# ThibHlln/smartpy

Measured on AMD Instinct MI355X. Metric: MC sample-timesteps/sec/GPU; 1e5 LHS x hourly 10-yr forcing, higher is better.
Workload: dtype f64

## Files before the change

### smartpy_amd/build.py

```python
import os
import shutil
import subprocess
import sys
from concurrent.futures import ThreadPoolExecutor

HERE = os.path.dirname(os.path.abspath(__file__))
CSRC = os.path.join(HERE, 'csrc')
LIB = os.path.join(CSRC, 'libsmart_amd.so')
ARCH = 'gfx950'

UNITS = {
    'smart_literal.hip': ['-ffp-contract=off'],
    'smart_fast_intervals.hip': ['-ffp-contract=fast-honor-pragmas', '-fno-honor-nans'],
    'smart_fast_runs.hip': ['-ffp-contract=fast-honor-pragmas', '-fno-honor-nans'],
    'smart_fast_steps.hip': ['-ffp-contract=fast-honor-pragmas', '-fno-honor-nans'],
    'smart_fast_reports.hip': ['-ffp-contract=fast-honor-pragmas', '-fno-honor-nans'],
    'smart_fast_guarded.hip': ['-ffp-contract=fast-honor-pragmas'],
    'smart_quantiles.hip': [],
    'smart_objfn_windows.hip': [],
    'smart_flow_duration.hip': [],
    'smart_signatures.hip': [],
    'smart_sobol.hip': [],
    'smart_bootstrap.hip': [],
    'smart_pareto.hip': [],
    'smart_ensemble_scores.hip': [],
    'smart_dynia.hip': [],
    'smart_pawn.hip': [],
    'smart_demcz.hip': ['-ffp-contract=off'],
    'smart_error_model.hip': ['-ffp-contract=off'],
    'smart_capi.hip': [],
    'smart_analysis_capi.hip': [],
    'smart_hostio.cpp': ['-pthread'],
}
COMMON = ['-O3', '-fPIC', '-std=c++17', '--offload-arch=' + ARCH, '-fno-gpu-rdc', '-Wall']
DEPS = sorted(f for f in os.listdir(CSRC) if f.endswith('.h')) + [os.path.join('..', '..', 'include', 'smart_amd.h')]


def hipcc():
    exe = shutil.which('hipcc') or '/opt/rocm/bin/hipcc'
    if not os.path.exists(exe):
        raise RuntimeError('hipcc not found: the HIP extension cannot be built')
    return exe


def _stale(target, sources):
    if not os.path.exists(target):
        return True
    t = os.path.getmtime(target)
    return any(os.path.getmtime(s) > t for s in sources)


def build(force=False, verbose=False, extra_flags=(), lib_path=LIB):
    cc = hipcc()
    deps = [os.path.join(CSRC, d) for d in DEPS] + [os.path.abspath(__file__)]
    objs, jobs = [], []
    suffix = '' if lib_path == LIB else '.' + os.path.basename(lib_path)
    for unit, flags in UNITS.items():
        src = os.path.join(CSRC, unit)
        obj = os.path.join(CSRC, os.path.splitext(unit)[0] + suffix + '.o')
        if force or _stale(obj, [src] + deps):
            jobs.append([cc] + COMMON + flags + list(extra_flags) + ['-c', src, '-o', obj])
        objs.append(obj)
    if jobs:
        if verbose:
            for cmd in jobs:
                print(' '.join(cmd))
        with ThreadPoolExecutor(max_workers=min(len(jobs), os.cpu_count() or 1)) as pool:
            list(pool.map(subprocess.check_call, jobs))
    from . import isa_lint
    relink = force or _stale(lib_path, objs)
    if relink or isa_lint.record_state(lib_path) != 'this-build':
        tmp = '%s.%d.tmp' % (lib_path, os.getpid())
        try:
            if relink:
                cmd = [cc, '-shared', '-fPIC', '-pthread', '--offload-arch=' + ARCH, '-o', tmp] + objs
                if verbose:
                    print(' '.join(cmd))
                subprocess.check_call(cmd)
            else:
                shutil.copy(lib_path, tmp)
            isa_lint.lint_and_record(tmp, record_for=lib_path, stamp=True, check=lambda path: lint(path, verbose))
            os.replace(tmp, lib_path)
        finally:
            if os.path.exists(tmp):
                os.remove(tmp)
    return lib_path


class BuildLintError(RuntimeError):
    pass


def lint(path, verbose=False):
    from . import isa_lint
    report = isa_lint.check_library(path)
    report['library'] = os.path.basename(LIB)
    if verbose or report['problems']:
# ... 11 lines not shown
```

### smartpy_amd/csrc/smart_capi.hip

```cpp
#include "smart_capi_internal.h"
#include "smart_fast_entry.h"

#include <cmath>
#include <cstdarg>
#include <cstdio>
#include <cstdlib>
#include <cstring>
#include <mutex>
#include <vector>

namespace smart {

static_assert(kStatusSliceTimeout == SMART_STATUS_SLICE_TIMEOUT && kStatusStalePlan == SMART_STATUS_STALE_PLAN,
              "status bits of smart_device.h and include/smart_amd.h");

static thread_local char g_err[512] = "";

int fail(int code, const char *fmt, ...)
{
    va_list ap;
    va_start(ap, fmt);
    vsnprintf(g_err, sizeof(g_err), fmt, ap);
    va_end(ap);
    return code;
// ... 56 lines not shown
                    r[4 * j + 1] = f[t].y;
                    r[4 * j + 2] = obs && dev && rr >= 0 && rr < a.R ? obs[rr] : 0.0;
                    r[4 * j + 3] = obs && dev && rr >= 0 && rr < a.R ? dev[rr] : 0.0;
                }
                code = a.gap == 1 ? every_code(p, step_kind(f[2 * p]), step_kind(f[2 * p + 1]))
                                  : gap_code(p, a.gap, step_kind(f[2 * p]), step_kind(f[2 * p + 1]));
            }
            for (int j = 0; j < 8; ++j)
                rec[p * 8 + j] = r[j];
            codes[p] = code;
        }
    }
    if (bad)
        __hip_atomic_fetch_or(a.fflags + blockIdx.y, bad, __ATOMIC_RELAXED, __HIP_MEMORY_SCOPE_AGENT);
    if (wild && a.hdr)
        __hip_atomic_fetch_or(a.hdr + kHdrStatus, kStatusNonFiniteForcing, __ATOMIC_RELAXED, __HIP_MEMORY_SCOPE_AGENT);
}

__global__ void smart_workspace_reset(int *hdr, long n_hdr, int *flags, long n_flags)
{
    const long i = (long)blockIdx.x * blockDim.x + threadIdx.x;
    if (i < n_hdr)
        hdr[i] = 0;
    if (i < n_flags)
        flags[i] = 0;
}

__global__ __launch_bounds__(kWave) void smart_classify_rows(KArgs a)
{
    const int cls = wave_class(a, (long)blockIdx.x, (long)blockIdx.y);
    if (threadIdx.x == 0) {
        __hip_atomic_fetch_or(a.hdr + kHdrPlan, 1 << cls, __ATOMIC_RELAXED, __HIP_MEMORY_SCOPE_AGENT);
        if (cls == 3)
            __hip_atomic_fetch_add(a.hdr + kHdrPlanIllCond, 1, __ATOMIC_RELAXED, __HIP_MEMORY_SCOPE_AGENT);
    }
}

__global__ void smart_classify_forcing(KArgs a, int *hdr)
{
    const long c = (long)blockIdx.x * blockDim.x + threadIdx.x;
    if (c < a.n_catch) {
        const int kind = forcing_kind(a, a.fflags[c]);
        __hip_atomic_fetch_or(hdr + kHdrPlan,
                              kind == kForcingIntervals ? SMART_PLAN_FORCING_PIECEWISE
                                                        : (kind == kForcingRuns ? SMART_PLAN_FORCING_RUNS
                                                                                : SMART_PLAN_FORCING_VARYING),
                              __ATOMIC_RELAXED, __HIP_MEMORY_SCOPE_AGENT);
    }
}

constexpr int kMaxDevices = 64, kMaxTodo = 8, kMaxAux = kMaxTodo - 1;

struct DeviceCtx {
    std::once_flag once;
    int n_simd = 0;
    std::mutex mu;
    hipStream_t aux[kMaxAux] = {};
    hipEvent_t fork = nullptr, join[kMaxAux] = {};
    size_t lds_size[kNumFastKernels][17] = {};
    bool lds_known[kNumFastKernels][17] = {};
};

static DeviceCtx g_dev[kMaxDevices];

static DeviceCtx *device_ctx()
{
    int dev = 0;
    if (hipGetDevice(&dev) != hipSuccess || dev < 0 || dev >= kMaxDevices)
        return nullptr;
    DeviceCtx *d = &g_dev[dev];
    std::call_once(d->once, [d, dev] {
        int cus = 0;
        if (hipDeviceGetAttribute(&cus, hipDeviceAttributeMultiprocessorCount, dev) == hipSuccess && cus > 0)
            d->n_simd = cus * 4;
    });
    return d->n_simd > 0 ? d : nullptr;
}

struct Overrides {
    int pair_blocks = -1;
    int time_slices = 0;
    int illcond_form = SMART_LITERAL_FORM_AUTO;
    bool taper = true;
    int exits = -1;
    long max_polls = kDefaultMaxPolls;
    int drop_slice = 0;
    bool allsteps_fast = false;
};

static Overrides read_overrides()
{
    Overrides o;
    if (const char *v = getenv("SMART_PAIR_BLOCKS"))
        o.pair_blocks = atoi(v) != 0;
    if (const char *v = getenv("SMART_TIME_SLICES"))
        o.time_slices = atoi(v) <= 0 ? 1 : atoi(v);
    if (const char *v = getenv("SMART_SLICE_TAPER"))
        o.taper = atoi(v) != 0;
    if (const char *v = getenv("SMART_ILLCOND_FORM"))
        o.illcond_form = !strcmp(v, "rows")    ? SMART_LITERAL_FORM_ROWS
                         : !strcmp(v, "lanes") ? SMART_LITERAL_FORM_LANES
                                               : SMART_LITERAL_FORM_AUTO;
    if (const char *v = getenv("SMART_EXITS"))
        o.exits = atoi(v) != 0;
    if (const char *v = getenv("SMART_DEBUG_MAX_POLLS"))
        o.max_polls = atol(v) > 0 ? atol(v) : kDefaultMaxPolls;
    if (const char *v = getenv("SMART_DEBUG_DROP_SLICE"))
        o.drop_slice = atoi(v);
    if (const char *v = getenv("SMART_ALLSTEPS_MATH"))
        o.allsteps_fast = !strcmp(v, "fast");
    return o;
}

struct FastKernelInfo {
    const void *handle;
    const char *name;
    int cls;
    bool sliced;
    int waves;
};

static const FastKernelInfo kFastKernels[kNumFastKernels] = {
#define X(id, symbol, cls, sliced, waves) {reinterpret_cast<const void *>(&symbol), #symbol, cls, sliced, waves},
    SMART_FAST_KERNELS(X)
#undef X
};

static size_t lds_for_residency(DeviceCtx *d, FastKernel k, int per_cu)
{
    if (per_cu < 1 || per_cu > 16)
        return 0;
    if (!d->lds_known[k][per_cu]) {
        size_t found = 0;
        for (size_t x = (size_t)(160 * 1024 / per_cu) / 256 * 256;
             x >= 1024 && x > (size_t)(160 * 1024 / (per_cu + 1)) - 2048; x -= 256) {
            int nb = 0;
            if (hipOccupancyMaxActiveBlocksPerMultiprocessor(&nb, kFastKernels[k].handle, kWave, x) != hipSuccess)
                break;
            if (nb == per_cu) {
                found = x;
                break;
            }
            if (nb > per_cu)
                break;
        }
        d->lds_size[k][per_cu] = found;
        d->lds_known[k][per_cu] = true;
    }
    return d->lds_size[k][per_cu];
}

static int merged_report(const SmartEnsemble *e);

extern "C" __attribute__((used, visibility("default"))) volatile char smart_lint_stamp[40] = "SMART_LINT_STAMP=unchecked";

static bool pair_blocks_wanted(const Overrides &ov)
{
    if (ov.pair_blocks >= 0)
        return ov.pair_blocks != 0;
    static const char ok[] = "SMART_LINT_STAMP=pairs-ok";
    for (size_t i = 0; i + 1 < sizeof(ok); ++i)
        if (smart_lint_stamp[i] != ok[i])
            return false;
    return true;
}

static bool uses_records(const SmartEnsemble *e)
{
    const int merged = merged_report(e);
    return merged == kReportEvery || ((merged == kReportMean || merged == kReportLast) && e->report_gap % kChunk != 0);
}

struct Layout {
    size_t header = 0;
    size_t stats_off = 0, stats = 0;
    size_t state_off = 0, state = 0;
    size_t flags_off = 0, flags = 0;
    size_t codes_off = 0, codes = 0;
    size_t ecodes_off = 0;
#ifdef SMART_SLICE_TIMELINE
    size_t timeline_off = 0, timeline = 0;
#endif
    size_t total = 0;
    size_t handover() const { return state + flags; }
};
// ... 303 lines not shown
    x.n_seg = plan_time_slices(e, d->n_simd, ov, &x.per_simd, &x.load);
    if (x.n_seg > 1 && !w.state)
        x.n_seg = 1;
    x.exits = ov.exits >= 0 ? ov.exits : x.load > 2.5;
    x.class_mask = plan & 0xf;
    if (plan & SMART_PLAN_CLASS_REGULAR) {
        if (x.intervals) {
            if (plan & SMART_PLAN_FORCING_PIECEWISE) {
                x.push(e->final_vars ? kIntervalsStates : (x.exits ? kIntervalsExits : kIntervals));
                x.pc_mask |= kPcIntervals;
            }
            if (plan & SMART_PLAN_FORCING_RUNS) {
                x.push(e->final_vars ? kRunsStates : (x.exits ? kRunsExits : kRuns));
                x.pc_mask |= kPcRuns;
            }
            if (plan & SMART_PLAN_FORCING_VARYING) {
                x.push(e->final_vars ? kStepsStates : kSteps);
                x.pc_mask |= kPcSteps;
            }
        } else if (x.report == kReportLast) {
            if (plan & SMART_PLAN_FORCING_PIECEWISE) {
                x.push(kIntervalsRaw);
                x.pc_mask |= kPcIntervals;
            }
            if (plan & (SMART_PLAN_FORCING_RUNS | SMART_PLAN_FORCING_VARYING)) {
                x.push(kStepsRaw);
                x.pc_mask |= kPcSteps | kPcRuns;
            }
        } else if (x.report == kReportEvery) {
            x.push(kStepsEvery);
            x.pc_mask = kPcIntervals | kPcSteps | kPcRuns;
        } else {
            x.push(kPlain);
        }
    }
    if (plan & SMART_PLAN_CLASS_STIFF)
        x.push(kStiff);
    if (plan & SMART_PLAN_CLASS_GUARD)
        x.push(kGuard);
    if (plan & SMART_PLAN_CLASS_ILLCOND) {
        x.illcond_blocks = count_illcond_blocks(e, plan);
        x.illcond_rows = illcond_form(e, d->n_simd, x.illcond_blocks, ov);
        x.push(x.illcond_rows ? kIllCond : kIllCondLanes);
    }
    if (x.overflow)
        return fail(SMART_E_SIZE, "internal: a call wants more than %d kernels", kMaxTodo);
    if (x.n_todo == 0)
        return fail(SMART_E_SIZE, "the plan names no class of rows");
    return SMART_OK;
}

static int run(const SmartEnsemble *e, const Overrides &ov, bool literal_rows = false)
{
    int rc = check(e);
    if (rc)
        return rc;
    if ((rc = device_ready()))
        return rc;
    hipStream_t s = (hipStream_t)e->stream;
    const Workspace w = carve(e, ov);
    KArgs a = kernel_args(e, w);

    if (e->objfn)
        hipLaunchKernelGGL(smart_obs_prepare, dim3((unsigned)e->n_catchments), dim3(256), 0, s, e->obs, a.R, w.stats);

    const dim3 grid((unsigned)a.n_blocks, (unsigned)e->n_catchments);
    if (e->math_mode == SMART_MATH_LITERAL) {
        if (w.hdr)
            reset_workspace(w, e->n_catchments, nullptr, 0, s);
        a.hdr = nullptr;
        launch_literal(a, grid, a.np_mean ? (size_t)a.gap * kWave * sizeof(double) : 0, s, literal_rows);
        HIP_TRY(hipGetLastError());
        return SMART_OK;
    }

    DeviceCtx *d = device_ctx();
    if (!d)
        return fail(SMART_E_NO_DEVICE, "cannot query the current HIP device");
    Decision x;
    if ((rc = decide(e, d, w, ov, &x)))
        return rc;
    const int n_seg = x.n_seg, n_todo = x.n_todo;
    a.exits = x.exits;
    a.class_mask = x.class_mask;
    a.pc_mask = x.pc_mask;

    KArgs a_sliced = a;
    if (n_seg > 1) {
        a_sliced.n_seg = n_seg;
        a_sliced.taper = ov.taper && slice_taper_applies(a.W / a.gap + a.R, n_seg);
        a_sliced.seg_state = (double *)w.state;
        a_sliced.seg_flag = (int *)(w.state + (w.lay.flags_off - w.lay.state_off));
        a_sliced.max_polls = ov.max_polls;
        a_sliced.debug_drop = ov.drop_slice;
#ifdef SMART_SLICE_TIMELINE
        a_sliced.timeline = (unsigned long long *)w.timeline;
#endif
    }
    if (w.hdr) {
        reset_workspace(w, e->n_catchments, a_sliced.seg_flag, n_seg > 1 ? a.seg_blocks : 0, s);
        scan_forcing(e, a, w, ov, s);
        if (x.report >= 0 && (x.class_mask & SMART_PLAN_CLASS_REGULAR)) {
            a.fflags = a_sliced.fflags = w.fflags;
            set_codes(&a, w, ov);
            a_sliced.codes = a.codes, a_sliced.estream = a.estream, a_sliced.ecodes = a.ecodes;
        }
    }

    std::lock_guard<std::mutex> lock(d->mu);
    auto launch = [&](FastKernel k, hipStream_t st) -> hipError_t {
        if (kFastKernels[k].sliced && n_seg > 1) {
            const size_t lds = x.per_simd <= 3 ? lds_for_residency(d, k, 4 * x.per_simd) : 0;
            return launch_kernel(k, a_sliced, dim3((unsigned)(a.seg_blocks * n_seg), 1), lds, st);
        }
        return launch_kernel(k, a, dim3(grid.x * kFastKernels[k].waves, grid.y), 0, st);
    };
    if (n_todo == 1) {
        HIP_TRY(launch(x.todo[0], s));
        return SMART_OK;
    }
    if (!d->fork) {
        HIP_TRY(hipEventCreateWithFlags(&d->fork, hipEventDisableTiming));
        for (int i = 0; i < kMaxAux; ++i) {
            HIP_TRY(hipStreamCreateWithFlags(&d->aux[i], hipStreamNonBlocking));
            HIP_TRY(hipEventCreateWithFlags(&d->join[i], hipEventDisableTiming));
        }
    }
    HIP_TRY(hipEventRecord(d->fork, s));
    for (int i = 1; i < n_todo; ++i) {
        HIP_TRY(hipStreamWaitEvent(d->aux[i - 1], d->fork, 0));
        HIP_TRY(launch(x.todo[i], d->aux[i - 1]));
        HIP_TRY(hipEventRecord(d->join[i - 1], d->aux[i - 1]));
    }
    HIP_TRY(launch(x.todo[0], s));
    for (int i = 1; i < n_todo; ++i)
        HIP_TRY(hipStreamWaitEvent(s, d->join[i - 1], 0));
    return SMART_OK;
}

static int describe(const SmartEnsemble *e, const Overrides &ov, char *text, int64_t len)
{
    if (!text || len < 1)
        return fail(SMART_E_NULL, "smart_describe_launch: no room for the text");
    text[0] = 0;
    int rc = check(e);
    if (rc)
        return rc;
    if (e->math_mode == SMART_MATH_LITERAL) {
        snprintf(text, (size_t)len, "smart_ensemble_literal");
        return SMART_OK;
    }
    if ((rc = device_ready()))
        return rc;
    DeviceCtx *d = device_ctx();
    if (!d)
        return fail(SMART_E_NO_DEVICE, "cannot query the current HIP device");
    Decision x;
    if ((rc = decide(e, d, carve(e, ov), ov, &x)))
        return rc;
    const long blocks = (e->n_samples + kWave - 1) / kWave * e->n_catchments;
    size_t used = 0;
    for (int i = 0; i < x.n_todo && used + 1 < (size_t)len; ++i) {
        const FastKernelInfo &k = kFastKernels[x.todo[i]];
        char *at = text + used;
        const size_t room = (size_t)len - used;
        int n;
// ... 419 lines not shown
```

### smartpy_amd/csrc/smart_device.h

```cpp
#pragma once

#include "smart_slice_cuts.h"
#include "smart_matrix_common.h"

#include <hip/hip_runtime.h>

#include <type_traits>

namespace smart {

constexpr int kMaxDiv = 12;
constexpr int kForcingInsane = 1 << 30;

struct KArgs {
    long N, T, W, gap, R, first_len;
    int report_type;
    int np_mean;
    double dt;
    const double *area;
    const double *forcing;
    const double *params;
    long pstride_c;
    const double *extra;
    const double *initial;
    const double *obs;
    const double *gw_obs;
    const double *ws;
    double *discharge;
    long ld;
    double *gw;
    double *objfn;
    double *final_vars;
    int exits = 1;
    int class_mask = 0xf;
    int pc_mask = 0x7;
    int *hdr = nullptr;
    int *fflags = nullptr;
    const double *estream = nullptr;
    const unsigned *ecodes = nullptr;
    int pair_stride = 0;
    const uint2 *codes = nullptr;
    int n_div = 0;
    int div[kMaxDiv] = {};
    int n_seg = 1;
    int taper = 0;
    long n_catch = 1;
    long n_blocks = 0;
    long seg_blocks = 0;
    double *seg_state = nullptr;
    int *seg_flag = nullptr;
    long max_polls = 0;
    int debug_drop = 0;
#ifdef SMART_SLICE_TIMELINE
    unsigned long long *timeline = nullptr;
#endif
};
#ifdef SMART_SLICE_TIMELINE
constexpr int kTimelineFields = 5, kTimelineSlices = 64;
__device__ __forceinline__ void timeline_note(const KArgs &a, long block, long c, int seg, int field,
                                              unsigned long long value)
{
    if (a.timeline && a.n_seg > 1 && seg < kTimelineSlices && seg < a.n_seg && threadIdx.x == 0)
        a.timeline[((long)seg * a.seg_blocks + c * a.n_blocks + block) * kTimelineFields + field] = value;
}
#endif

enum SegField : int {
    kSegState = 0,
    kSegDenRaw = 13,
    kSegPend = 15,
    kSegOutflows = 16,
    kSegA = 17,
    kSegB,
    kSegC1,
    kSegC2,
    kSegC3,
    kSegShift,
    kSegFields
};
enum HdrInt : int {
    kHdrStatus = 0,
    kHdrTicket = 1,
    kHdrPlan = 8,
    kHdrPlanIllCond = 9,
    kHdrInts = 64
};
constexpr int kStatusSliceTimeout = 1, kStatusStalePlan = 2, kStatusNonFiniteForcing = 4;

__device__ __forceinline__ void raise_status(const KArgs &a, int bit)
{
    if (a.hdr && threadIdx.x == 0)
        __hip_atomic_fetch_or(a.hdr + kHdrStatus, bit, __ATOMIC_RELAXED, __HIP_MEMORY_SCOPE_AGENT);
}

#define SMART_NOPS_0 ""
#define SMART_NOPS_1 "s_nop 0\n\t"
#define SMART_NOPS_2 SMART_NOPS_1 SMART_NOPS_1
#define SMART_NOPS_4 SMART_NOPS_2 SMART_NOPS_2
#define SMART_NOPS_8 SMART_NOPS_4 SMART_NOPS_4
#define SMART_NOPS_3 SMART_NOPS_2 SMART_NOPS_1
#define SMART_NOPS_5 SMART_NOPS_4 SMART_NOPS_1
#define SMART_NOPS_6 SMART_NOPS_4 SMART_NOPS_2
#define SMART_NOPS_7 SMART_NOPS_4 SMART_NOPS_3
#define SMART_NOPS_9 SMART_NOPS_8 SMART_NOPS_1
#define SMART_NOPS_10 SMART_NOPS_8 SMART_NOPS_2
#define SMART_NOPS_11 SMART_NOPS_8 SMART_NOPS_3
#define SMART_NOPS_12 SMART_NOPS_8 SMART_NOPS_4
#define SMART_NOPS_13 SMART_NOPS_8 SMART_NOPS_5
#define SMART_NOPS_14 SMART_NOPS_8 SMART_NOPS_6
#define SMART_NOPS_15 SMART_NOPS_8 SMART_NOPS_7
#define SMART_NOPS_(n) SMART_NOPS_##n
#define SMART_NOPS(n) SMART_NOPS_(n)
#define SMART_PLACE_LOOP(phase) asm volatile(".p2align 6\n\t" SMART_NOPS(phase))
#ifndef SMART_STEPS_PHASE
#define SMART_STEPS_PHASE 1
#endif
#ifndef SMART_PS_STRIDE
#define SMART_PS_STRIDE 2368
// ... 844 lines not shown
__device__ __forceinline__ Work claim_work(const KArgs &a, int sliced_kernel)
{
    Work w;
    if (a.n_seg > 1) {
        unsigned t = 0;
        if (threadIdx.x == 0)
            t = __hip_atomic_fetch_add(reinterpret_cast<unsigned *>(a.hdr) + kHdrTicket + sliced_kernel, 1u,
                                       __ATOMIC_RELAXED, __HIP_MEMORY_SCOPE_AGENT);
        t = (unsigned)__builtin_amdgcn_readfirstlane((int)t);
        const long slot = (long)(t % (unsigned long)a.seg_blocks);
        w.seg = (int)(t / (unsigned long)a.seg_blocks);
        w.c = slot / a.n_blocks;
        w.block = slot % a.n_blocks;
    } else {
        w.block = blockIdx.x;
        w.c = blockIdx.y;
        w.seg = 0;
    }
    return w;
}

__device__ __forceinline__ bool wait_for_slice(const KArgs &a, long slot, int seg)
{
    int *flag = a.seg_flag + slot;
    long polls = 0;
    int v;
    while ((v = __hip_atomic_load(flag, __ATOMIC_RELAXED, __HIP_MEMORY_SCOPE_AGENT)) > -seg && v < seg) {
        __builtin_amdgcn_s_sleep(kPollSleep);
        if (++polls > a.max_polls) {
            raise_status(a, kStatusSliceTimeout);
            return false;
        }
    }
    __builtin_amdgcn_fence(__ATOMIC_ACQUIRE, "agent");
    return v >= seg;
}

__device__ __forceinline__ void publish_slice(const KArgs &a, long slot, int seg, bool good)
{
    asm volatile("s_waitcnt vmcnt(0)" ::: "memory");
    __builtin_amdgcn_fence(__ATOMIC_RELEASE, "agent");
    asm volatile("s_waitcnt vmcnt(0)" ::: "memory");
    if (threadIdx.x == 0)
        __hip_atomic_store(a.seg_flag + slot, good ? seg + 1 : -(seg + 1), __ATOMIC_RELAXED, __HIP_MEMORY_SCOPE_AGENT);
}

constexpr int kReportMean = 0, kReportLast = 1, kReportEvery = 2;

template <class Model, int FORCING, int REPORT = kReportMean>
__device__ __forceinline__ void run_ensemble_merged(const KArgs &a, const double2 *__restrict__ forcing,
                                                    const double *__restrict__ obs_all,
                                                    const double *__restrict__ ws_all, long block, long catchment,
                                                    int seg, int fflags)
{
    constexpr bool piecewise = FORCING != kForcingVarying;
    constexpr bool runs = FORCING == kForcingRuns;
    static_assert(REPORT == kReportMean || (!Model::kSplit && !runs), "raw / every-step reports: merged model, no runs");
    static_assert(REPORT != kReportEvery || !piecewise, "a report every step is a step loop");
    static_assert(Model::kStateFields <= kSegPend, "the model's states end in front of the other hand-over fields");
    const LaneCtx x = lane_ctx(a, block, catchment);
    const long slot = catchment * a.n_blocks + block;
    Model m;
    init_model(a, x, m);
    const long gap = a.gap;
    const long run_len = runs ? run_length(a, fflags) : gap;
    if constexpr (piecewise)
        m.setup_intervals(REPORT == kReportLast ? run_len - 1 : run_len);
    const double2 *__restrict__ f = forcing + x.c * a.T;

    int fits = 0;
    unsigned not_quick = ~0u;
    if constexpr (piecewise && Model::kWetAsm) {
        m.note_capacity();
        const bool fits_b = m.over_mask == 0;
        fits = __builtin_amdgcn_readfirstlane((int)fits_b);
        not_quick = 0u - (unsigned)__builtin_amdgcn_readfirstlane((int)!(fits_b && !(fflags & kForcingInsane)));
        asm("" : "+s"(fits), "+s"(not_quick));
    }
    auto no_bits = [](double x, unsigned unless = 0) {
        unsigned long long b = __builtin_bit_cast(unsigned long long, x) | unless;
        asm("" : "+s"(b));
        return b == 0;
    };
    auto interval = [&](const double2 v, double &acc, double &num, double &den) {
        if constexpr (piecewise && Model::kWetAsm) {
            if (no_bits(v.x, not_quick)) {
                if (no_bits(v.y)) {
                    m.calm_interval(run_len, acc);
                } else {
                    m.dry_interval(-v.y, run_len, acc);
                }
                return;
            }
        }
        const double ex = m.excess(v.x, v.y);
        if (ex < 0.0) {
            m.dry_interval(ex, run_len, acc);
        } else {
            if constexpr (piecewise && Model::kWetAsm)
                m.wet_interval(ex, run_len, acc, num, den, fits);
            else
                m.wet_interval(ex, run_len, acc, num, den);
        }
    };

    [[maybe_unused]] auto interval_last = [&](const double2 v, double &qo, double &qg, double &qi) {
        if constexpr (piecewise && REPORT == kReportLast && Model::kWetAsm) {
            double sink = 0.0, n0 = 0.0, n1 = 0.0;
            if (no_bits(v.x, not_quick)) {
                if (no_bits(v.y)) {
                    m.calm_interval(gap - 1, sink);
                    m.last_step_flows(qo, qg, qi);
                    m.calm_interval(1, sink);
                } else {
                    m.dry_interval_last(-v.y, gap, qo, qg, qi);
                }
                return;
            }
            const double ex = m.excess(v.x, v.y);
            if (ex < 0.0) {
                m.dry_interval_last(ex, gap, qo, qg, qi);
            } else {
                m.wet_interval(ex, gap - 1, sink, n0, n1, fits);
                m.last_step_flows(qo, qg, qi);
                m.wet_interval(ex, 1, sink, n0, n1, fits);
            }
        }
    };

    const long n_warm = a.W / gap, n_all = n_warm + a.R;
    const long g0 = a.taper ? slice_cut_tapered(n_all, seg, a.n_seg) : n_all * seg / a.n_seg;
    const long g1 = a.taper ? slice_cut_tapered(n_all, seg + 1, a.n_seg) : n_all * (seg + 1) / a.n_seg;
    const long wa = g0 < n_warm ? g0 : n_warm, wb = g1 < n_warm ? g1 : n_warm;
    const long ra = g0 > n_warm ? g0 - n_warm : 0, rb = g1 > n_warm ? g1 - n_warm : 0;
    const bool last = seg == a.n_seg - 1;

    Reporter rep;
    rep.init(a, x, obs_all, ws_all);
    [[maybe_unused]] const double *__restrict__ obs_c = obs_all ? obs_all + x.c * a.R : nullptr;
    [[maybe_unused]] const double *__restrict__ dev_c = ws_all ? ws_all + x.c * (kWsHead + a.R) + kWsHead : nullptr;
    [[maybe_unused]] const uint2 *codes_c = a.codes ? a.codes + x.c * code_chunks(a.T) : nullptr;
    [[maybe_unused]] const double2 *f_asm = reinterpret_cast<const double2 *>(a.forcing) + x.c * a.T;
    double num = 0.0, den = 0.0, q_out_total = 0.0;
    [[maybe_unused]] double num_raw = 0.0, den_raw = 0.0;
    double *hand = a.seg_state + (slot * kSegFields) * kWave + x.lane;
    if (seg > 0) {
        if (!wait_for_slice(a, slot, seg)) {
            const double nan = quiet_nan();
            if (a.discharge && x.live)
                for (long r = ra; r < rb; ++r)
                    a.discharge[(x.c * a.R + r) * a.ld + x.n] = nan;
            if (last) {
                if (x.live) {
                    a.gw[x.c * a.N + x.n] = nan;
                    if (a.objfn)
                        for (int i = 0; i < 8; ++i)
                            a.objfn[(x.c * a.N + x.n) * 8 + i] = nan;
                    if (a.final_vars)
                        for (int i = 0; i < 19; ++i)
                            a.final_vars[(x.c * a.N + x.n) * 19 + i] = nan;
                }
            } else {
                publish_slice(a, slot, seg, false);
            }
            return;
        }
#ifdef SMART_SLICE_TIMELINE
        timeline_note(a, block, catchment, seg, 3, __builtin_amdgcn_s_memrealtime());
#endif
        m.load_state(hand, kWave);
        if constexpr (REPORT == kReportLast) {
            num_raw = hand[kSegOutflows * kWave];
            den_raw = hand[kSegDenRaw * kWave];
        } else {
            q_out_total = hand[kSegOutflows * kWave];
        }
        rep.A = hand[kSegA * kWave];
        rep.B = hand[kSegB * kWave];
        rep.C1 = hand[kSegC1 * kWave];
        rep.C2 = hand[kSegC2 * kWave];
        rep.C3 = hand[kSegC3 * kWave];
        rep.shift = hand[kSegShift * kWave];
    }

    double *const park = Model::kSplit ? a.final_vars + (x.c * a.N + x.n) * 19 : nullptr;
    auto park_state = [&]() {
        if constexpr (Model::kSplit) {
            m.save_state(park, 1);
            if constexpr (!piecewise)
                park[15] = m.pend;
        }
    };

    double s0 = 0.0, s1 = 0.0, s2 = 0.0;
    const double inv_gap = 1.0 / (double)gap;
    const bool starts_run = ra == 0 && (rb > 0 || last);
    constexpr bool deferring = !piecewise;
    [[maybe_unused]] const int n_lead = (int)(rep.r1 + 1 > ra ? (rep.r1 + 1 < rb ? rep.r1 + 1 - ra : rb - ra) : 0);
    [[maybe_unused]] int store = __builtin_amdgcn_readfirstlane((int)(a.discharge != nullptr));
    asm("" : "+s"(store));
    [[maybe_unused]] const int k_park = Model::kSplit && ra <= a.R - 1 && a.R - 1 < rb ? (int)(a.R - 1 - ra) : -1;
    if constexpr (piecewise)
        rep.begin_rows(a, x, ra);
    if constexpr (runs) {
        const long per = gap / run_len;
        interval_loop(f, wa * per, wb * per, run_len, [&](int, const double2 v) { interval(v, s0, s1, s2); });
        if (starts_run)
            m.begin_run();
// ... 318 lines not shown
```

### smartpy_amd/csrc/smart_fast_model.h

```cpp
#pragma once

#include "smart_device.h"
#include "smart_fast_arms.h"

namespace smart {

template <bool STIFF, bool GUARD, bool MERGE = false, bool EXITS = true, bool SPLIT = false>
struct FastModel {
    static_assert(!(MERGE && STIFF), "the clamps of structure.py:429-450 act on each reservoir separately");
    static_assert(MERGE || !SPLIT, "SPLIT refines the merged form");
    static constexpr bool kExactDivide = false;
    static constexpr bool kSplit = SPLIT;

    double pT, pC, pD, hz, sz, z;
    double dec_s, dec_f, dec_g, cq_s, cq_f, cq_g;
    double a_r, inv_a_r;
    double a_s, a_f, a_g;
    double car_s, car_f, car_g, om_ar;
    double k_s, k_f, k_g, k_r, mm_to_m3;
    double l0, l1, l2, l3, l4, l5;
    double u_ove, u_dra, u_int, u_sgw, u_dgw, u_riv;
    double q_out, q_in, q_gw;

    __device__ void setup(double area, double dt, const double *p)
// ... 288 lines not shown
        l1 = fma(-l1, s1 * 0.5, l1);
        l2 = fma(-l2, s1 * (1.0 / 3.0), l2);
        l3 = fma(-l3, s1 * 0.25, l3);
        l4 = fma(-l4, s1 * 0.2, l4);
        l5 = fma(-l5, s1 * (1.0 / 6.0), l5);
        const double deep = SPLIT ? deep_leak(s1, p2, p3, p4, p5, p6) : 0.0;
        l0 = fma(-l0, p6, l0);
        l1 = fma(-l1, p5, l1);
        l2 = fma(-l2, p4, l2);
        l3 = fma(-l3, p3, l3);
        l4 = fma(-l4, p2, l4);
        l5 = fma(-l5, s1, l5);
        const double inf = (tot - after_int) + fma(-pD, rem, ex_in);
        fma_in_place(u_ove, dec_s, fma(pD, rem, e_h * tot));
        fma_in_place(u_int, dec_f, inf);
        const double upper = (l0 + l1) + (l2 + l3), lower = l4 + l5;
        asm("v_add_f64 %0, %1, %2" : "+v"(tot) : "v"(upper), "v"(lower));
        const double xg = after_int - tot;
        fma_in_place(u_sgw, dec_g, xg);
        if (SPLIT) {
            fma_in_place(u_dra, dec_s, pD * rem);
            fma_in_place(u_dgw, dec_g, deep);
        }
        if (kBalanceSums)
            xg_sum += xg;
    }

#ifndef SMART_WET_ASM
#define SMART_WET_ASM 1
#endif
    static constexpr bool kWetAsm = SMART_WET_ASM && kLeakBalance && !kExits && !SPLIT && !STIFF;

    __device__ __forceinline__ void calm_interval(long n, double &acc)
    {
        static_assert(kWetAsm, "calm_interval() is the asm loop of the straight-line merged kernels");
        double tot = layer_sum();
        double t0, t1, xf, xg, w_s1, w_p2, w_p3, w_p4, w_p5, w_p6, w_ai;
        int cnt;
        asm volatile(SMART_A_CALM_INTERVAL
                     : [l0] "+v"(l0), [l1] "+v"(l1), [l2] "+v"(l2), [l3] "+v"(l3), [l4] "+v"(l4), [l5] "+v"(l5),
                       [ys] "+v"(u_ove), [yf] "+v"(u_int), [yg] "+v"(u_sgw), [riv] "+v"(u_riv), [acc] "+v"(acc),
                       [tot] "+v"(tot), [xgs] "+v"(xg_sum), [t0] "=&v"(t0), [t1] "=&v"(t1), [xf] "=&v"(xf),
                       [xg] "=&v"(xg), [s1] "=&v"(w_s1), [p2] "=&v"(w_p2), [p3] "=&v"(w_p3), [p4] "=&v"(w_p4),
                       [p5] "=&v"(w_p5), [p6] "=&v"(w_p6), [ai] "=&v"(w_ai), [cnt] "=&s"(cnt)
                     : [cs] "v"(car_s), [cf] "v"(car_f), [cg] "v"(car_g), [oma] "v"(om_ar), [ds] "v"(dec_s),
                       [df] "v"(dec_f), [dg] "v"(dec_g), [sz] "v"(sz), [k3] "s"(-(1.0 / 3.0)), [k5] "s"(-0.2),
                       [k6] "s"(-(1.0 / 6.0)), [n] "s"((int)n)
                     : "scc");
    }

    __device__ __forceinline__ void wet_interval(double ex, long n, double &acc, double &num, double &den,
                                                 const int fits = 0)
    {
        if constexpr (kWetAsm) {
            const double e_h = ex * hz;
            double tot = layer_sum();
            double t0, t1, xs, xf, xg, w_s1, w_p2, w_p3, w_p4, w_p5, w_p6, w_ai;
            int cnt;
            asm volatile(SMART_A_WET_INTERVAL
                         : [l0] "+v"(l0), [l1] "+v"(l1), [l2] "+v"(l2), [l3] "+v"(l3), [l4] "+v"(l4), [l5] "+v"(l5),
                           [ys] "+v"(u_ove), [yf] "+v"(u_int), [yg] "+v"(u_sgw), [riv] "+v"(u_riv), [acc] "+v"(acc),
                           [tot] "+v"(tot), [xgs] "+v"(xg_sum), [t0] "=&v"(t0), [t1] "=&v"(t1), [xs] "=&v"(xs),
                           [xf] "=&v"(xf), [xg] "=&v"(xg), [s1] "=&v"(w_s1), [p2] "=&v"(w_p2), [p3] "=&v"(w_p3),
                           [p4] "=&v"(w_p4), [p5] "=&v"(w_p5), [p6] "=&v"(w_p6), [ai] "=&v"(w_ai), [cnt] "=&s"(cnt)
                         : [cs] "v"(car_s), [cf] "v"(car_f), [cg] "v"(car_g), [oma] "v"(om_ar), [ds] "v"(dec_s),
                           [df] "v"(dec_f), [dg] "v"(dec_g), [sz] "v"(sz), [z] "v"(z), [pd] "v"(pD), [ex] "v"(ex),
                           [eh] "v"(e_h), [k3] "s"(-(1.0 / 3.0)), [k5] "s"(-0.2), [k6] "s"(-(1.0 / 6.0)),
                           [n] "s"((int)n), [ok] "s"(fits)
                         : "scc", "vcc");
        } else if (kLeakBalance) {
            const double e_h = ex * hz;
            double tot = layer_sum();
#pragma unroll 1
            for (long k = 0; k < n; ++k) {
                route_and_sum(acc, num, den);
                wet_balance(ex, e_h, tot);
            }
        } else {
            for (long k = 0; k < n; ++k) {
                route_and_sum(acc, num, den);
                wet_lanes(ex);
            }
        }
    }

    __device__ __forceinline__ void dry_lanes(double ex)
    {
        double d = -ex;
        dry(l0, d, pC);
        auto handed_down = [](double x) { return GUARD ? x != 0.0 : x > 0.0; };
        if (__builtin_amdgcn_ballot_w64(handed_down(d)) != 0) {
            dry(l1, d, pC);
            if (__builtin_amdgcn_ballot_w64(handed_down(d)) != 0) {
                dry(l2, d, pC);
                dry(l3, d, pC);
                dry(l4, d, pC);
                dry(l5, d, pC);
            }
        }
        u_ove = clamp(u_ove * dec_s);
        u_int = clamp(u_int * dec_f);
        u_sgw = clamp(u_sgw * dec_g);
        if (!MERGE || SPLIT) {
            u_dra = clamp(u_dra * dec_s);
            u_dgw = clamp(u_dgw * dec_g);
        }
    }

    __device__ __forceinline__ void route_and_sum(double &acc, double &num, double &den)
    {
        double q_r = u_riv;
        double u_new;
        if (MERGE && !STIFF && kBalanceSums) {
            q_out = u_riv;
            q_gw = cq_g * u_sgw;
            q_in = fma(cq_s, u_ove, fma(cq_f, u_int, q_gw));
            const double y = fma(car_s, u_ove, fma(car_f, u_int, car_g * u_sgw));
            if (kExits) {
                sum_then_fma_in_place(acc, u_riv, om_ar, y);
            } else {
                acc += u_riv;
                fma_in_place(u_riv, om_ar, y);
            }
            return;
        }
        if (MERGE) {
            u_new = u_riv;
            fma_in_place(u_new, om_ar, fma(car_s, u_ove, fma(car_f, u_int, car_g * u_sgw)));
            q_gw = cq_g * u_sgw;
            q_in = fma(cq_s, u_ove, fma(cq_f, u_int, q_gw));
        } else {
            q_gw = u_sgw + u_dgw;
            q_in = ((u_ove + u_dra) + u_int) + q_gw;
            u_new = fma(q_in - u_riv, a_r, u_riv);
        }
        if (STIFF) {
            if (u_new < 0.0) {
                q_r = 0.95 * fma(u_riv, inv_a_r, q_in);
                u_new = fma(q_in - q_r, a_r, u_riv);
            }
        }
        u_riv = u_new;
        q_out = q_r;
        acc += q_r;
        if (!kBalanceSums) {
            num += q_gw;
            den += q_in;
        }
    }

    static constexpr int kStateFields = 15;

    __device__ void save_state(double *p, int stride) const
    {
        const double v[kStateFields] = {l0, l1, l2, l3, l4, l5, u_ove, u_int, u_sgw, u_riv, g0, r0, xg_sum, u_dra, u_dgw};
#pragma unroll
        for (int i = 0; i < (SPLIT ? 15 : 13); ++i)
            p[i * stride] = v[i];
    }

    __device__ void load_state(const double *p, int stride)
    {
        double v[kStateFields] = {};
#pragma unroll
        for (int i = 0; i < (SPLIT ? 15 : 13); ++i)
            v[i] = p[i * stride];
// ... 513 lines not shown
```

### smartpy_amd/csrc/smart_fast_reports.hip

```cpp
#include "smart_fast_entry.h"

namespace smart {

SMART_FAST_KERNEL(smart_fast_steps_raw) { merged_kernel<FastModel<false, false, true>, kForcingVarying, kReportLast>(a, forcing, obs, ws); }

SMART_FAST_KERNEL(smart_fast_intervals_raw)
{
    merged_kernel<FastModel<false, false, true, false>, kForcingIntervals, kReportLast>(a, forcing, obs, ws);
}

SMART_FAST_KERNEL(smart_fast_steps_every) { merged_kernel<FastModel<false, false, true>, kForcingVarying, kReportEvery>(a, forcing, obs, ws); }

}
```

### smartpy_amd/csrc/smart_fast_runs.hip

```cpp
#include "smart_fast_entry.h"

namespace smart {

SMART_FAST_KERNEL(smart_fast_runs_exits) { merged_kernel<FastModel<false, false, true, true>, kForcingRuns>(a, forcing, obs, ws); }

SMART_FAST_KERNEL(smart_fast_runs) { merged_kernel<FastModel<false, false, true, false>, kForcingRuns>(a, forcing, obs, ws); }

SMART_FAST_KERNEL(smart_fast_runs_states)
{
    merged_kernel<FastModel<false, false, true, true, true>, kForcingRuns>(a, forcing, obs, ws);
}

}
```

Before: 959.6 billion.

## Make wet/dry interval branching wave-uniform with twin-state merge for mixed waves

Replaces the per-lane wet/dry branch in the runs and interval-last paths with a wave ballot. Uniform waves take a single path, and mixed waves run both paths on a copied model state and select per lane. The runs and intervals_raw kernels are moved into their own compile units built with an LLVM flag that skips structurizing uniform regions, aiming for cleaner scalar control flow. The cost is that mixed waves execute both branches, and register pressure rises from the twin model copy.

After: 959.4 billion. No clear change (-0.0%).

```diff
diff --git a/smartpy_amd/build.py b/smartpy_amd/build.py
--- a/smartpy_amd/build.py
+++ b/smartpy_amd/build.py
@@ -9,10 +9,14 @@
 LIB = os.path.join(CSRC, 'libsmart_amd.so')
 ARCH = 'gfx950'
 
+UNIFORM_AS_IS = ['-mllvm', '-structurizecfg-skip-uniform-regions']
+
 UNITS = {
     'smart_literal.hip': ['-ffp-contract=off'],
     'smart_fast_intervals.hip': ['-ffp-contract=fast-honor-pragmas', '-fno-honor-nans'],
-    'smart_fast_runs.hip': ['-ffp-contract=fast-honor-pragmas', '-fno-honor-nans'],
+    'smart_fast_runs.hip': ['-ffp-contract=fast-honor-pragmas', '-fno-honor-nans'] + UNIFORM_AS_IS,
+    'smart_fast_intervals_raw.hip': ['-ffp-contract=fast-honor-pragmas', '-fno-honor-nans'] + UNIFORM_AS_IS,
+    'smart_fast_runs_variants.hip': ['-ffp-contract=fast-honor-pragmas', '-fno-honor-nans'],
     'smart_fast_steps.hip': ['-ffp-contract=fast-honor-pragmas', '-fno-honor-nans'],
     'smart_fast_reports.hip': ['-ffp-contract=fast-honor-pragmas', '-fno-honor-nans'],
     'smart_fast_guarded.hip': ['-ffp-contract=fast-honor-pragmas'],
diff --git a/smartpy_amd/csrc/smart_capi.hip b/smartpy_amd/csrc/smart_capi.hip
--- a/smartpy_amd/csrc/smart_capi.hip
+++ b/smartpy_amd/csrc/smart_capi.hip
@@ -162,6 +162,7 @@
     int time_slices = 0;
     int illcond_form = SMART_LITERAL_FORM_AUTO;
     bool taper = true;
+    bool wet_uniform = true;
     int exits = -1;
     long max_polls = kDefaultMaxPolls;
     int drop_slice = 0;
@@ -181,6 +182,8 @@
         o.illcond_form = !strcmp(v, "rows")    ? SMART_LITERAL_FORM_ROWS
                          : !strcmp(v, "lanes") ? SMART_LITERAL_FORM_LANES
                                                : SMART_LITERAL_FORM_AUTO;
+    if (const char *v = getenv("SMART_WET_UNIFORM"))
+        o.wet_uniform = atoi(v) != 0;
     if (const char *v = getenv("SMART_EXITS"))
         o.exits = atoi(v) != 0;
     if (const char *v = getenv("SMART_DEBUG_MAX_POLLS"))
@@ -650,6 +653,7 @@
         return rc;
     const int n_seg = x.n_seg, n_todo = x.n_todo;
     a.exits = x.exits;
+    a.wet_uniform = ov.wet_uniform;
     a.class_mask = x.class_mask;
     a.pc_mask = x.pc_mask;
 
diff --git a/smartpy_amd/csrc/smart_device.h b/smartpy_amd/csrc/smart_device.h
--- a/smartpy_amd/csrc/smart_device.h
+++ b/smartpy_amd/csrc/smart_device.h
@@ -34,6 +34,7 @@
     int exits = 1;
     int class_mask = 0xf;
     int pc_mask = 0x7;
+    int wet_uniform = 1;
     int *hdr = nullptr;
     int *fflags = nullptr;
     const double *estream = nullptr;
@@ -1044,6 +1045,11 @@
         asm("" : "+s"(b));
         return b == 0;
     };
+    [[maybe_unused]] const unsigned long long all_lanes = __builtin_amdgcn_ballot_w64(true);
+    [[maybe_unused]] unsigned long long per_lane = a.wet_uniform ? 0ull : ~0ull;
+    [[maybe_unused]] auto no_lanes = [&](unsigned long long mask) {
+        return (mask | per_lane) == 0;
+    };
     auto interval = [&](const double2 v, double &acc, double &num, double &den) {
         if constexpr (piecewise && Model::kWetAsm) {
             if (no_bits(v.x, not_quick)) {
@@ -1056,7 +1062,27 @@
             }
         }
         const double ex = m.excess(v.x, v.y);
-        if (ex < 0.0) {
+        if constexpr (runs && Model::kWetAsm) {
+            const bool dry_lane = ex < 0.0;
+            const unsigned long long dry = __builtin_amdgcn_ballot_w64(dry_lane);
+            if (no_lanes(dry ^ all_lanes)) {
+                m.dry_interval(ex, run_len, acc);
+            } else {
+                const bool mixed = !no_lanes(dry);
+                Model d;
+                double acc_d;
+                if (__builtin_expect(mixed, 0)) {
+                    d = m.twin();
+                    acc_d = Model::own_copy(acc);
+                }
+                m.wet_interval(ex, run_len, acc, num, den, fits);
+                if (__builtin_expect(mixed, 0)) {
+                    d.dry_interval(ex, run_len, acc_d);
+                    m.keep_lanes(dry_lane, d);
+                    acc = dry_lane ? acc_d : acc;
+                }
+            }
+        } else if (ex < 0.0) {
             m.dry_interval(ex, run_len, acc);
         } else {
             if constexpr (piecewise && Model::kWetAsm)
@@ -1080,12 +1106,24 @@
                 return;
             }
             const double ex = m.excess(v.x, v.y);
-            if (ex < 0.0) {
+            const bool dry_lane = ex < 0.0;
+            const unsigned long long dry = __builtin_amdgcn_ballot_w64(dry_lane);
+            if (no_lanes(dry ^ all_lanes)) {
                 m.dry_interval_last(ex, gap, qo, qg, qi);
             } else {
+                const bool mixed = !no_lanes(dry);
+                Model d;
+                if (__builtin_expect(mixed, 0))
+                    d = m.twin();
                 m.wet_interval(ex, gap - 1, sink, n0, n1, fits);
                 m.last_step_flows(qo, qg, qi);
                 m.wet_interval(ex, 1, sink, n0, n1, fits);
+                if (__builtin_expect(mixed, 0)) {
+                    double qo_d, qg_d, qi_d;
+                    d.dry_interval_last(ex, gap, qo_d, qg_d, qi_d);
+                    m.keep_lanes(dry_lane, d);
+                    qo = dry_lane ? qo_d : qo, qg = dry_lane ? qg_d : qg, qi = dry_lane ? qi_d : qi;
+                }
             }
         }
     };
diff --git a/smartpy_amd/csrc/smart_fast_intervals_raw.hip b/smartpy_amd/csrc/smart_fast_intervals_raw.hip
--- /dev/null
+++ b/smartpy_amd/csrc/smart_fast_intervals_raw.hip
@@ -0,0 +1,10 @@
+#include "smart_fast_entry.h"
+
+namespace smart {
+
+SMART_FAST_KERNEL(smart_fast_intervals_raw)
+{
+    merged_kernel<FastModel<false, false, true, false>, kForcingIntervals, kReportLast>(a, forcing, obs, ws);
+}
+
+}
diff --git a/smartpy_amd/csrc/smart_fast_model.h b/smartpy_amd/csrc/smart_fast_model.h
--- a/smartpy_amd/csrc/smart_fast_model.h
+++ b/smartpy_amd/csrc/smart_fast_model.h
@@ -394,6 +394,30 @@
                 wet_lanes(ex);
             }
         }
+    }
+
+    static __device__ __forceinline__ double own_copy(double x)
+    {
+        double c;
+        asm("v_mov_b64 %0, %1" : "=v"(c) : "v"(x));
+        return c;
+    }
+    __device__ __forceinline__ auto twin() const
+    {
+        auto w = *this;
+        w.l0 = own_copy(l0), w.l1 = own_copy(l1), w.l2 = own_copy(l2);
+        w.l3 = own_copy(l3), w.l4 = own_copy(l4), w.l5 = own_copy(l5);
+        w.u_ove = own_copy(u_ove), w.u_int = own_copy(u_int), w.u_sgw = own_copy(u_sgw);
+        w.u_riv = own_copy(u_riv), w.xg_sum = own_copy(xg_sum);
+        return w;
+    }
+    template <class Other>
+    __device__ __forceinline__ void keep_lanes(bool theirs, const Other &w)
+    {
+        l0 = theirs ? w.l0 : l0, l1 = theirs ? w.l1 : l1, l2 = theirs ? w.l2 : l2;
+        l3 = theirs ? w.l3 : l3, l4 = theirs ? w.l4 : l4, l5 = theirs ? w.l5 : l5;
+        u_ove = theirs ? w.u_ove : u_ove, u_int = theirs ? w.u_int : u_int, u_sgw = theirs ? w.u_sgw : u_sgw;
+        u_riv = theirs ? w.u_riv : u_riv, xg_sum = theirs ? w.xg_sum : xg_sum;
     }
 
     __device__ __forceinline__ void dry_lanes(double ex)
diff --git a/smartpy_amd/csrc/smart_fast_reports.hip b/smartpy_amd/csrc/smart_fast_reports.hip
--- a/smartpy_amd/csrc/smart_fast_reports.hip
+++ b/smartpy_amd/csrc/smart_fast_reports.hip
@@ -4,11 +4,6 @@
 
 SMART_FAST_KERNEL(smart_fast_steps_raw) { merged_kernel<FastModel<false, false, true>, kForcingVarying, kReportLast>(a, forcing, obs, ws); }
 
-SMART_FAST_KERNEL(smart_fast_intervals_raw)
-{
-    merged_kernel<FastModel<false, false, true, false>, kForcingIntervals, kReportLast>(a, forcing, obs, ws);
-}
-
 SMART_FAST_KERNEL(smart_fast_steps_every) { merged_kernel<FastModel<false, false, true>, kForcingVarying, kReportEvery>(a, forcing, obs, ws); }
 
 }
diff --git a/smartpy_amd/csrc/smart_fast_runs.hip b/smartpy_amd/csrc/smart_fast_runs.hip
--- a/smartpy_amd/csrc/smart_fast_runs.hip
+++ b/smartpy_amd/csrc/smart_fast_runs.hip
@@ -2,13 +2,6 @@
 
 namespace smart {
 
-SMART_FAST_KERNEL(smart_fast_runs_exits) { merged_kernel<FastModel<false, false, true, true>, kForcingRuns>(a, forcing, obs, ws); }
-
 SMART_FAST_KERNEL(smart_fast_runs) { merged_kernel<FastModel<false, false, true, false>, kForcingRuns>(a, forcing, obs, ws); }
 
-SMART_FAST_KERNEL(smart_fast_runs_states)
-{
-    merged_kernel<FastModel<false, false, true, true, true>, kForcingRuns>(a, forcing, obs, ws);
 }
-
-}
diff --git a/smartpy_amd/csrc/smart_fast_runs_variants.hip b/smartpy_amd/csrc/smart_fast_runs_variants.hip
--- /dev/null
+++ b/smartpy_amd/csrc/smart_fast_runs_variants.hip
@@ -0,0 +1,12 @@
+#include "smart_fast_entry.h"
+
+namespace smart {
+
+SMART_FAST_KERNEL(smart_fast_runs_exits) { merged_kernel<FastModel<false, false, true, true>, kForcingRuns>(a, forcing, obs, ws); }
+
+SMART_FAST_KERNEL(smart_fast_runs_states)
+{
+    merged_kernel<FastModel<false, false, true, true, true>, kForcingRuns>(a, forcing, obs, ws);
+}
+
+}
```
